# Copojacaab/APDA-FFT

Hardware: NVIDIA B200
Metric: FFT+peak windows/sec at N=4096 (higher is better)
Workload: dtype f32

## Files before the change

apda-fft_b200/csrc/fft_f32_fast.cu:

```cuda
#include <mutex>

#include "fft_f32_fast.cuh"

namespace {

template <int N, int CENTER, bool FULL, bool HALF_OUT>
__global__ void __launch_bounds__(Plan<N>::WPB *(N / 32), Plan<N>::MINB)
fft_f32_fast_kernel(const float *__restrict__ samples, int n_samples, int64_t ld, int64_t batch,
                    const float2 *__restrict__ tw1,
                    const float2 *__restrict__ twu,
                    float2 *__restrict__ spec, const int *__restrict__ nv) {
    using P = Plan<N>;
    constexpr int M = N / 2, R1 = P::R1, R2 = P::R2, R3 = P::R3, T = M / 16, WPB = P::WPB;
    constexpr int S1 = R2 * R3;
    constexpr int LD = S1 + 16 / R1;
    static_assert(R1 * R2 * R3 == M, "plan");
    __shared__ __align__(16) float2 sm[WPB][R1 * LD];
    __shared__ uint32_t sel[WPB][64];
    __shared__ float red[WPB][8];

    const int wslot = threadIdx.x / T;
    const int t = threadIdx.x % T;
    const int64_t win = (int64_t)blockIdx.x * WPB + wslot;
    if (win >= batch) return;
    if (nv && nv[win] != n_samples) return;
    const int64_t winc = win;
    float2 *s = sm[wslot];

    k1_forward<N, CENTER, FULL>(samples, n_samples, ld, winc, tw1, s, sel[wslot], red[wslot], wslot, t);

    float4 *out = reinterpret_cast<float4 *>(spec + win * (int64_t)N);
    const float4 *s4 = reinterpret_cast<const float4 *>(s);
    const float4 *twu4 = reinterpret_cast<const float4 *>(twu);
#pragma unroll
    for (int g = 0; g < (M / 2) / T; ++g) {
        const int p = t + T * g;
        const float4 zk = s4[p];
        const float2 za = s[(M - 2 * p) & (M - 1)];
        const float2 zb = s[M - 2 * p - 1];
        const float4 w = __ldg(twu4 + p);
        const float2 cj = make_float2(1.f, -1.f), ncj = make_float2(-1.f, 1.f), hf = make_float2(0.5f, 0.5f);
        const float2 zk0 = make_float2(zk.x, zk.y), zk1 = make_float2(zk.z, zk.w);
        const float2 s0 = pfma(za, cj, zk0), d0 = pfma(za, ncj, zk0);
        const float2 s1 = pfma(zb, cj, zk1), d1 = pfma(zb, ncj, zk1);
        const float2 t0 = cmul(d0, make_float2(w.x, w.y)), t1 = cmul(d1, make_float2(w.z, w.w));
        const float2 x0 = pfma(s0, hf, t0), x1 = pfma(s1, hf, t1);
        float4 lo4 = make_float4(x0.x, x0.y, x1.x, x1.y);
        if (p == 0) lo4.x = lo4.y = 0.f;
        out[p] = lo4;
        if (!HALF_OUT) {
            const float2 y0 = pfma(s0, hf, make_float2(-t0.x, -t0.y)), y1 = pfma(s1, hf, make_float2(-t1.x, -t1.y));
            out[M / 2 + p] = make_float4(y0.x, y0.y, y1.x, y1.y);
        }
    }
}

struct FastTables {
    float2 *tw1 = nullptr, *twu = nullptr;
};

}

struct FastCache {
    std::map<int64_t, FastTables> tabs;
};
static std::map<apda_ctx *, FastCache> g_fast;
static std::mutex g_fast_mu;
static FastCache &fast_cache_of(apda_ctx *ctx) {
    std::lock_guard<std::mutex> lock(g_fast_mu);
    return g_fast[ctx];
}

template <int N>
static int fast_tables(apda_ctx *ctx, FastTables *out) {
    using P = Plan<N>;
    constexpr int M = N / 2, R1 = P::R1, R2 = P::R2, R3 = P::R3, S1 = R2 * R3;
    auto &cache = fast_cache_of(ctx).tabs;
    auto it = cache.find(N);
    if (it != cache.end()) {
        *out = it->second;
        return APDA_OK;
    }
    const double two_pi = 6.283185307179586476925286766559;
    std::vector<float2> h1((size_t)R1 * S1), hu(M), h2((size_t)R2 * R3);
    for (int k1 = 0; k1 < R1; ++k1)
        for (int c = 0; c < S1; ++c) {
            const double a = -two_pi * (double)((int64_t)k1 * c % M) / (double)M;
            h1[(size_t)k1 * S1 + c] = make_float2((float)cos(a), (float)sin(a));
        }
    for (int k = 0; k < M; ++k) {
        const double a = -two_pi * (double)k / (double)N;
        hu[k] = make_float2((float)(0.5 * sin(a)), (float)(-0.5 * cos(a)));
    }
    for (int k2 = 0; k2 < R2; ++k2)
        for (int n3 = 0; n3 < R3; ++n3) {
            const double a = -two_pi * (double)(k2 * n3) / (double)(R2 * R3);
            h2[(size_t)k2 * R3 + n3] = make_float2((float)cos(a), (float)sin(a));
        }
    FastTables ft;
    APDA_CUDA(cudaMalloc(&ft.tw1, h1.size() * sizeof(float2)));
    APDA_CUDA(cudaMalloc(&ft.twu, hu.size() * sizeof(float2)));
    APDA_CUDA(cudaMemcpy(ft.tw1, h1.data(), h1.size() * sizeof(float2), cudaMemcpyHostToDevice));
    APDA_CUDA(cudaMemcpy(ft.twu, hu.data(), hu.size() * sizeof(float2), cudaMemcpyHostToDevice));
    const void *sym = N == 1024 ? (const void *)c_tw2_1024 : N == 2048 ? (const void *)c_tw2_2048
                    : N == 4096 ? (const void *)c_tw2_4096 : (const void *)c_tw2_8192;
    APDA_CUDA(cudaMemcpyToSymbol(sym, h2.data(), h2.size() * sizeof(float2)));
    cache[N] = ft;
    *out = ft;
    return APDA_OK;
}

template <int N>
static int launch_fast_n(apda_ctx *ctx, cudaStream_t st, const float *d_samples, int64_t n_samples, int64_t ld,
                         int64_t batch, int flags, float *d_spec, const int *d_nv, bool half_out) {
    using P = Plan<N>;
    FastTables ft;
    APDA_TRY(fast_tables<N>(ctx, &ft));
    const int threads = P::WPB * (N / 32);
    const int64_t blocks = (batch + P::WPB - 1) / P::WPB;
    const bool full = n_samples == N && (reinterpret_cast<uintptr_t>(d_samples) & 7u) == 0 && (ld & 1) == 0;
    void (*kern)(const float *, int, int64_t, int64_t, const float2 *, const float2 *, float2 *, const int *);
#define APDA_K1(C, F) (half_out ? fft_f32_fast_kernel<N, C, F, true> : fft_f32_fast_kernel<N, C, F, false>)
    kern = flags == APDA_CENTER_MEDIAN ? (full ? APDA_K1(APDA_CENTER_MEDIAN, true) : APDA_K1(APDA_CENTER_MEDIAN, false))
           : flags == APDA_CENTER_MEAN ? (full ? APDA_K1(APDA_CENTER_MEAN, true) : APDA_K1(APDA_CENTER_MEAN, false))
                                       : (full ? APDA_K1(APDA_CENTER_NONE, true) : APDA_K1(APDA_CENTER_NONE, false));
#undef APDA_K1
    kern<<<(unsigned)blocks, threads, 0, st>>>(d_samples, (int)n_samples, ld, batch, ft.tw1, ft.twu,
                                               reinterpret_cast<float2 *>(d_spec), d_nv);
    ctx->launches++;
    APDA_CUDA(cudaGetLastError());
    return APDA_OK;
}

int fft_f32_fast_get_tables(apda_ctx *ctx, int64_t N, const float2 **tw1, const float2 **twu) {
    FastTables ft;
    switch (N) {
        case 1024: APDA_TRY(fast_tables<1024>(ctx, &ft)); break;
        case 2048: APDA_TRY(fast_tables<2048>(ctx, &ft)); break;
        case 4096: APDA_TRY(fast_tables<4096>(ctx, &ft)); break;
        case 8192: APDA_TRY(fast_tables<8192>(ctx, &ft)); break;
        default: apda_set_error("fft_f32_fast: unsupported N=%lld", (long long)N); return APDA_ERR_UNSUPPORTED;
    }
    *tw1 = ft.tw1;
    *twu = ft.twu;
    return APDA_OK;
}

bool fft_f32_fast_supports(int64_t N) { return N == 1024 || N == 2048 || N == 4096 || N == 8192; }

int launch_fft_f32_fast(apda_ctx *ctx, cudaStream_t st, const float *d_samples, int64_t n_samples, int64_t ld,
                        int64_t batch, int64_t N, int flags, float *d_spec, const int *d_nv, bool half_out) {
    switch (N) {
        case 1024: return launch_fast_n<1024>(ctx, st, d_samples, n_samples, ld, batch, flags, d_spec, d_nv, half_out);
        case 2048: return launch_fast_n<2048>(ctx, st, d_samples, n_samples, ld, batch, flags, d_spec, d_nv, half_out);
        case 4096: return launch_fast_n<4096>(ctx, st, d_samples, n_samples, ld, batch, flags, d_spec, d_nv, half_out);
        case 8192: return launch_fast_n<8192>(ctx, st, d_samples, n_samples, ld, batch, flags, d_spec, d_nv, half_out);
    }
    apda_set_error("fft_f32_fast: unsupported N=%lld", (long long)N);
    return APDA_ERR_UNSUPPORTED;
}

void fft_f32_fast_release(apda_ctx *ctx) {
    std::lock_guard<std::mutex> lock(g_fast_mu);
    auto it = g_fast.find(ctx);
    if (it == g_fast.end()) return;
    for (auto &kv : it->second.tabs) {
        cudaFree(kv.second.tw1);
        cudaFree(kv.second.twu);
    }
    g_fast.erase(it);
}
```

apda-fft_b200/csrc/fft_f32_fast.cuh:

```cuda
#pragma once
#include "common.cuh"

namespace {

__device__ __forceinline__ unsigned long long &u64(float2 &v) { return reinterpret_cast<unsigned long long &>(v); }
__device__ __forceinline__ const unsigned long long &u64(const float2 &v) {
    return reinterpret_cast<const unsigned long long &>(v);
}
__device__ __forceinline__ float2 cadd(float2 a, float2 b) {
    float2 r;
    asm("add.rn.f32x2 %0, %1, %2;" : "=l"(u64(r)) : "l"(u64(a)), "l"(u64(b)));
    return r;
}
__device__ __forceinline__ float2 csub(float2 a, float2 b) {
    float2 r;
    asm("sub.rn.f32x2 %0, %1, %2;" : "=l"(u64(r)) : "l"(u64(a)), "l"(u64(b)));
    return r;
}
__device__ __forceinline__ float2 pmul(float2 a, float2 b) {
    float2 r;
    asm("mul.rn.f32x2 %0, %1, %2;" : "=l"(u64(r)) : "l"(u64(a)), "l"(u64(b)));
    return r;
}
__device__ __forceinline__ float2 pfma(float2 a, float2 b, float2 c) {
    float2 r;
    asm("fma.rn.f32x2 %0, %1, %2, %3;" : "=l"(u64(r)) : "l"(u64(a)), "l"(u64(b)), "l"(u64(c)));
    return r;
}
__device__ __forceinline__ float2 cmul(float2 a, float2 w) {
    return make_float2(fmaf(a.x, w.x, -a.y * w.y), fmaf(a.x, w.y, a.y * w.x));
}

#define SQRT1_2f 0.70710678118654752440f
#define COS_PI_8f 0.92387953251128675613f
#define SIN_PI_8f 0.38268343236508977173f

__device__ __forceinline__ void add_sub_mi(float2 u, float2 d, float2 &plus, float2 &minus) {
    plus = make_float2(u.x + d.y, u.y - d.x);
    minus = make_float2(u.x - d.y, u.y + d.x);
}

__device__ __forceinline__ void fft4(float2 &a0, float2 &a1, float2 &a2, float2 &a3) {
    const float2 t0 = cadd(a0, a2), t1 = csub(a0, a2), t2 = cadd(a1, a3), d = csub(a1, a3);
    a0 = cadd(t0, t2);
    a2 = csub(t0, t2);
    add_sub_mi(t1, d, a1, a3);
}
__device__ __forceinline__ void fft8(float2 *v) {
    float2 e0 = v[0], e1 = v[2], e2 = v[4], e3 = v[6];
    float2 o0 = v[1], o1 = v[3], o2 = v[5], o3 = v[7];
    fft4(e0, e1, e2, e3);
    fft4(o0, o1, o2, o3);
    o1 = pmul(make_float2(o1.x + o1.y, o1.y - o1.x), make_float2(SQRT1_2f, SQRT1_2f));
    o3 = pmul(make_float2(o3.y - o3.x, o3.x + o3.y), make_float2(SQRT1_2f, -SQRT1_2f));
    v[0] = cadd(e0, o0);
    v[4] = csub(e0, o0);
    v[1] = cadd(e1, o1);
    v[5] = csub(e1, o1);
    add_sub_mi(e2, o2, v[2], v[6]);
    v[3] = cadd(e3, o3);
    v[7] = csub(e3, o3);
}
__device__ __forceinline__ void fft16(float2 *v) {
    float2 e[8], o[8];
#pragma unroll
    for (int i = 0; i < 8; ++i) {
        e[i] = v[2 * i];
        o[i] = v[2 * i + 1];
    }
    fft8(e);
    fft8(o);
    const float2 w1 = make_float2(COS_PI_8f, -SIN_PI_8f), w3 = make_float2(SIN_PI_8f, -COS_PI_8f);
    const float2 w5 = make_float2(-SIN_PI_8f, -COS_PI_8f), w7 = make_float2(-COS_PI_8f, -SIN_PI_8f);
    o[1] = cmul(o[1], w1);
    o[2] = pmul(make_float2(o[2].x + o[2].y, o[2].y - o[2].x), make_float2(SQRT1_2f, SQRT1_2f));
    o[3] = cmul(o[3], w3);
    o[5] = cmul(o[5], w5);
    o[6] = pmul(make_float2(o[6].y - o[6].x, o[6].x + o[6].y), make_float2(SQRT1_2f, -SQRT1_2f));
    o[7] = cmul(o[7], w7);
#pragma unroll
    for (int i = 0; i < 8; ++i) {
        if (i == 4) {
            add_sub_mi(e[4], o[4], v[4], v[12]);
        } else {
            v[i] = cadd(e[i], o[i]);
            v[i + 8] = csub(e[i], o[i]);
        }
    }
}
template <int R>
__device__ __forceinline__ void fft_r(float2 *v) {
    if (R == 16) fft16(v);
    else if (R == 8) fft8(v);
    else fft4(v[0], v[1], v[2], v[3]);
}

__constant__ float2 c_tw2_1024[64];
__constant__ float2 c_tw2_2048[64];
__constant__ float2 c_tw2_4096[128];
__constant__ float2 c_tw2_8192[256];
template <int N>
__device__ __forceinline__ const float2 *const_tw2() {
    return N == 1024 ? c_tw2_1024 : N == 2048 ? c_tw2_2048 : N == 4096 ? c_tw2_4096 : c_tw2_8192;
}

#ifndef APDA_K1_MINB_2048
#define APDA_K1_MINB_2048 8
#endif
#ifndef APDA_K1_MINB_1024
#define APDA_K1_MINB_1024 8
#endif
#ifndef APDA_K1_MINB_8192
#define APDA_K1_MINB_8192 4
#endif
#ifndef APDA_K1_MINB
#define APDA_K1_MINB 9
#endif
template <int N>
struct Plan;
template <>
struct Plan<8192> { static constexpr int R1 = 16, R2 = 16, R3 = 16, WPB = 1, MINB = APDA_K1_MINB_8192; };
template <>
struct Plan<4096> { static constexpr int R1 = 16, R2 = 16, R3 = 8, WPB = 1, MINB = APDA_K1_MINB; };
template <>
struct Plan<2048> { static constexpr int R1 = 16, R2 = 8, R3 = 8, WPB = 2, MINB = APDA_K1_MINB_2048; };
template <>
struct Plan<1024> { static constexpr int R1 = 8, R2 = 8, R3 = 8, WPB = 4, MINB = APDA_K1_MINB_1024; };

template <int T>
__device__ __forceinline__ void group_sync(int slot) {
    if (T == 32) __syncwarp();
    else if (slot == 0) asm volatile("bar.sync 1, %0;" ::"n"(T) : "memory");
    else asm volatile("bar.sync 2, %0;" ::"n"(T) : "memory");
}

__device__ __forceinline__ float next_above(float v) {
    float n = key_value(ordered_key(v) + 1u, 0.f);
    if (!(n > v)) n = key_value(ordered_key(v) + 2u, 0.f);
    return n;
}

__device__ __noinline__ float2 bracket_minmax(float2 a0, float2 a1, float2 a2, float2 a3, float2 a4, float2 a5, float2 a6,
                                              float2 a7, float2 a8, float2 a9, float2 a10, float2 a11, float2 a12, float2 a13,
                                              float2 a14, float2 a15, unsigned inb) {
    const float2 a[16] = {a0, a1, a2, a3, a4, a5, a6, a7, a8, a9, a10, a11, a12, a13, a14, a15};
    float vmin = CUDART_INF_F, vmax = -CUDART_INF_F;
#pragma unroll
    for (int i = 0; i < 16; ++i) {
        if (inb & (0x80000000u >> (2 * i))) {
            vmin = fminf(vmin, a[i].x);
            vmax = fmaxf(vmax, a[i].x);
        }
        if (inb & (0x80000000u >> (2 * i + 1))) {
            vmin = fminf(vmin, a[i].y);
            vmax = fmaxf(vmax, a[i].y);
        }
    }
#pragma unroll
    for (int o = 16; o > 0; o >>= 1) {
        vmin = fminf(vmin, __shfl_xor_sync(0xffffffffu, vmin, o));
        vmax = fmaxf(vmax, __shfl_xor_sync(0xffffffffu, vmax, o));
    }
    return make_float2(vmin, vmax);
}

constexpr int kTightenFrom = 4;
template <int T, bool FULL, typename Reload>
__device__ float select_median(const float2 (&v2)[16], int n_valid, uint32_t *sh , int t, int slot,
                               Reload reload ) {
#define VAL(i) (((i) & 1) ? v2[(i) >> 1].y : v2[(i) >> 1].x)
    constexpr int NW = (T + 31) / 32;
    const int lane = t & 31, warp = t >> 5;
    const int r_lo = (n_valid - 1) >> 1, r_hi = n_valid >> 1;
    float *shf = reinterpret_cast<float *>(sh);

    {
        float s1 = 0.f, s2 = 0.f;
        int cntv = 0;
#pragma unroll
        for (int c = 0; c < 16; c += 4) {
#pragma unroll
            for (int h = 0; h < 2; ++h) {
                const float raw = h ? v2[c].y : v2[c].x;
                const bool ok = FULL || raw < CUDART_INF_F;
                const float x = ok ? raw : 0.f;
                s1 += x;
                s2 = fmaf(x, x, s2);
                cntv += ok;
            }
        }
#pragma unroll
        for (int o = 16; o > 0; o >>= 1) {
            s1 += __shfl_xor_sync(0xffffffffu, s1, o);
            s2 += __shfl_xor_sync(0xffffffffu, s2, o);
        }
        if (!FULL) cntv = __reduce_add_sync(0xffffffffu, cntv);
        if (lane == 0) {
            shf[warp] = s1;
            shf[8 + warp] = s2;
            if (!FULL) sh[16 + warp] = (uint32_t)cntv;
        }
        if (t == 0) sh[48] = 0;
    }
    group_sync<T>(slot);
    float mean, sd;
    {
        float s1 = 0.f, s2 = 0.f;
        int cntv = FULL ? 8 * T : 0;
#pragma unroll
        for (int w = 0; w < NW; ++w) {
            s1 += shf[w];
            s2 += shf[8 + w];
            if (!FULL) cntv += (int)sh[16 + w];
        }
        const float inv = rcp_approx((float)max(cntv, 1));
        mean = s1 * inv;
        sd = sqrt_approx(fmaxf(fmaf(-mean, mean, s2 * inv), 0.f));
    }
    const float inv_density = fmaxf(2.5f * sd, 1e-30f) * rcp_approx((float)n_valid);

    float lo = -CUDART_INF_F, hi = CUDART_INF_F;
    int c_lo = 0, c_hi = n_valid;
    unsigned mask_lo = 0u, mask_hi = 0xffffffffu;
    if (!FULL) {
        mask_hi = 0u;
#pragma unroll
        for (int i = 0; i < 32; ++i) mask_hi = (mask_hi << 1) | (VAL(i) < CUDART_INF_F ? 1u : 0u);
    }
    float pivot = mean;
    for (int round = 0;; ++round) {
        if (round > 0) {
            if (c_hi - c_lo <= 32) break;
            if (round >= kTightenFrom) {
                const float2 mm = bracket_minmax(v2[0], v2[1], v2[2], v2[3], v2[4], v2[5], v2[6], v2[7], v2[8], v2[9], v2[10],
                                                 v2[11], v2[12], v2[13], v2[14], v2[15], ~mask_lo & mask_hi);
                if (lane == 0) {
                    shf[warp] = mm.x;
                    shf[8 + warp] = mm.y;
                }
                group_sync<T>(slot);
                float vmin = shf[0], vmax = shf[8];
#pragma unroll
                for (int w = 1; w < NW; ++w) {
                    vmin = fminf(vmin, shf[w]);
                    vmax = fmaxf(vmax, shf[8 + w]);
                }
                if (vmin == vmax) {
                    group_sync<T>(slot);
                    return vmin;
                }
                lo = vmin;
                hi = next_above(vmax);
            }
            const float lo_next = lo > -CUDART_INF_F ? next_above(lo) : -3.4028234e38f;
            if (!(lo_next < hi)) break;
            const float want = (float)r_lo + 0.5f;
            if (lo == -CUDART_INF_F) {
                pivot = hi - 1.5f * fmaxf((float)c_hi - want, 1.f) * inv_density * (float)(1 << min(round - 1, 20));
            } else if (hi == CUDART_INF_F) {
                pivot = lo + 1.5f * fmaxf(want - (float)c_lo, 1.f) * inv_density * (float)(1 << min(round - 1, 20));
            } else if (round % 3 == 2) {
                const uint32_t a = ordered_key(lo), b = ordered_key(hi);
                pivot = key_value(a + ((b - a) >> 1), 0.f);
            } else {
                pivot = lo + (hi - lo) * __fdividef(want - (float)c_lo, (float)(c_hi - c_lo));
            }
            if (!(pivot > lo)) pivot = lo_next;
            if (!(pivot < hi)) pivot = lo_next;
        }
        unsigned signs = 0;
        const float2 pv = make_float2(pivot, pivot);
#pragma unroll
        for (int i = 0; i < 16; ++i) {
            const float2 d = csub(v2[i], pv);
            signs = __funnelshift_l(__float_as_uint(d.x), signs, 1);
            signs = __funnelshift_l(__float_as_uint(d.y), signs, 1);
        }
        int cnt = __popc(signs);
        cnt = __reduce_add_sync(0xffffffffu, cnt);
        uint32_t *cslot = sh + 32 + 8 * (round & 1);
        if (lane == 0) cslot[warp] = (uint32_t)cnt;
        group_sync<T>(slot);
        int tot = 0;
#pragma unroll
        for (int w = 0; w < NW; ++w) tot += (int)cslot[w];
        if (tot <= r_lo) {
            lo = pivot;
            c_lo = tot;
            mask_lo = signs;
        } else if (tot > r_hi) {
            hi = pivot;
            c_hi = tot;
            mask_hi = signs;
        } else {
            float below = -CUDART_INF_F, above = CUDART_INF_F;
#pragma unroll
            for (int i = 0; i < 32; ++i) {
                if (VAL(i) < pivot) below = fmaxf(below, VAL(i));
                else above = fminf(above, VAL(i));
            }
#pragma unroll
            for (int o = 16; o > 0; o >>= 1) {
                below = fmaxf(below, __shfl_xor_sync(0xffffffffu, below, o));
                above = fminf(above, __shfl_xor_sync(0xffffffffu, above, o));
            }
            if (lane == 0) {
                shf[warp] = below;
                shf[8 + warp] = above;
            }
            group_sync<T>(slot);
#pragma unroll
            for (int w = 0; w < NW; ++w) {
                below = fmaxf(below, shf[w]);
                above = fminf(above, shf[8 + w]);
            }
            group_sync<T>(slot);
            return (below + above) * 0.5f;
        }
    }
    if (c_hi - c_lo > 32) {
        group_sync<T>(slot);
        return lo;
    }
    for (unsigned inb = ~mask_lo & mask_hi; inb; ) {
        const int q = __clz(inb);
        inb &= ~(0x80000000u >> q);
        const uint32_t pos = atomicAdd(&sh[48], 1u);
        if (pos < 32u) shf[pos] = reload(q);
    }
    group_sync<T>(slot);
    const int cnt = (int)sh[48];
    if (warp == 0) {
        float med;
        if (cnt > 32) {
            med = lo;
        } else {
            const float mine = lane < cnt ? shf[lane] : CUDART_INF_F;
            int rank = 0;
            for (int j = 0; j < cnt; ++j) {
                const float other = shf[j];
                rank += (other < mine) || (other == mine && j < lane);
            }
            const uint32_t m_lo = __ballot_sync(0xffffffffu, lane < cnt && rank == r_lo - c_lo);
            const uint32_t m_hi = __ballot_sync(0xffffffffu, lane < cnt && rank == r_hi - c_lo);
            const float a = __shfl_sync(0xffffffffu, mine, __ffs(m_lo) - 1);
            const float b = __shfl_sync(0xffffffffu, mine, __ffs(m_hi) - 1);
            med = (a + b) * 0.5f;
        }
        if (lane == 0) shf[49] = med;
    }
    group_sync<T>(slot);
    return shf[49];
}
#undef VAL

template <int N, int CENTER, bool FULL, int PF_AHEAD = 0>
__device__ __forceinline__ void k1_forward(const float *__restrict__ samples, const int n_samples, const int64_t ld,
                                           const int64_t winc, const float2 *__restrict__ tw1, float2 *s, uint32_t *sel_w,
                                           float *red_w, const int wslot, const int t, const int64_t pf_batch = 0) {
    constexpr int center = CENTER;
    using P = Plan<N>;
    constexpr int M = N / 2, R1 = P::R1, R2 = P::R2, R3 = P::R3, T = M / 16;
    constexpr int S1 = R2 * R3;
    constexpr int LD = S1 + 16 / R1;
    constexpr int G1 = 16 / R1, G2 = 16 / R2, G3 = 16 / R3;
    float2 v[16];
    const float *x = samples + winc * ld;
    const float2 *z = reinterpret_cast<const float2 *>(x);
    const bool full = FULL;
#pragma unroll
    for (int g = 0; g < G1; ++g) {
        const int c = t + T * g;
#pragma unroll
        for (int n1 = 0; n1 < R1; ++n1) {
            const int zi = n1 * S1 + c;
            float2 val;
            if (FULL) {
                val = __ldg(z + zi);
            } else {
                val.x = (2 * zi < n_samples) ? __ldg(x + 2 * zi) : 0.f;
                val.y = (2 * zi + 1 < n_samples) ? __ldg(x + 2 * zi + 1) : 0.f;
            }
            v[g * R1 + n1] = val;
        }
    }
    if (APDA_L2_PREFETCH && PF_AHEAD > 0) {
        const int64_t wn = winc + (int64_t)sm_count_reg() * PF_AHEAD;
        if (wn < pf_batch) l2_prefetch_span(samples + wn * ld, n_samples * (int)sizeof(float), t, T);
    }
    float shift = 0.f;
    if (center == APDA_CENTER_MEDIAN) {
        if (!full) {
#pragma unroll
            for (int g = 0; g < G1; ++g)
#pragma unroll
                for (int n1 = 0; n1 < R1; ++n1) {
                    const int zi = n1 * S1 + t + T * g;
                    if (2 * zi >= n_samples) v[g * R1 + n1].x = CUDART_INF_F;
                    if (2 * zi + 1 >= n_samples) v[g * R1 + n1].y = CUDART_INF_F;
                }
        }
        auto reload = [&](int q) {
            const int j = q >> 1;
            return __ldg(x + 2 * ((j % R1) * S1 + t + T * (j / R1)) + (q & 1));
        };
        shift = select_median<T, FULL>(v, n_samples, sel_w, t, wslot, reload);
        if (!full) {
#pragma unroll
            for (int i = 0; i < 16; ++i) {
                if (v[i].x == CUDART_INF_F) v[i].x = 0.f;
                if (v[i].y == CUDART_INF_F) v[i].y = 0.f;
            }
        }
    } else if (center == APDA_CENTER_MEAN) {
        float acc = 0.f;
#pragma unroll
        for (int i = 0; i < 16; ++i) acc += v[i].x + v[i].y;
#pragma unroll
        for (int o = 16; o > 0; o >>= 1) acc += __shfl_xor_sync(0xffffffffu, acc, o);
        if ((t & 31) == 0) red_w[t >> 5] = acc;
        group_sync<T>(wslot);
        float tot = 0.f;
#pragma unroll
        for (int w = 0; w < (T + 31) / 32; ++w) tot += red_w[w];
        shift = tot / (float)n_samples;
    }
#pragma unroll
    for (int g = 0; g < G1; ++g) {
        const int c = t + T * g;
        if (center != APDA_CENTER_NONE) {
#pragma unroll
            for (int n1 = 0; n1 < R1; ++n1) {
                const int zi = n1 * S1 + c;
                if (full) {
                    v[g * R1 + n1] = csub(v[g * R1 + n1], make_float2(shift, shift));
                } else {
                    if (2 * zi < n_samples) v[g * R1 + n1].x -= shift;
                    if (2 * zi + 1 < n_samples) v[g * R1 + n1].y -= shift;
                }
            }
        }
        fft_r<R1>(v + g * R1);
        s[c] = v[g * R1];
#pragma unroll
        for (int k1 = 1; k1 < R1; ++k1) s[k1 * LD + c] = cmul(v[g * R1 + k1], __ldg(tw1 + k1 * S1 + c));
    }
    group_sync<T>(wslot);

    const float2 *tw2 = const_tw2<N>();
#pragma unroll
    for (int g = 0; g < G2; ++g) {
        const int w = t + T * g;
        const int k1 = w % R1, n3 = w / R1;
        float2 *col = s + k1 * LD + n3;
#pragma unroll
        for (int n2 = 0; n2 < R2; ++n2) v[g * R2 + n2] = col[n2 * R3];
        fft_r<R2>(v + g * R2);
        col[0] = v[g * R2];
#pragma unroll
        for (int k2 = 1; k2 < R2; ++k2) col[k2 * R3] = cmul(v[g * R2 + k2], tw2[k2 * R3 + n3]);
    }
    group_sync<T>(wslot);

#pragma unroll
    for (int g = 0; g < G3; ++g) {
        const int w = t + T * g;
        const int k1 = w % R1, k2 = w / R1;
        const float2 *row = s + k1 * LD + k2 * R3;
#pragma unroll
        for (int n3 = 0; n3 < R3; ++n3) v[g * R3 + n3] = row[n3];
        fft_r<R3>(v + g * R3);
    }
    group_sync<T>(wslot);
#pragma unroll
    for (int g = 0; g < G3; ++g) {
        const int w = t + T * g;
#pragma unroll
        for (int k3 = 0; k3 < R3; ++k3) s[w + R1 * R2 * k3] = v[g * R3 + k3];
    }
    group_sync<T>(wslot);

}

}
```

apda-fft_b200/csrc/fused_f32.cu:

```cuda
#include <mutex>

#include "fft_f32_fast.cuh"
#include "peaks_fast.cuh"

int fft_f32_fast_get_tables(apda_ctx *ctx, int64_t N, const float2 **tw1, const float2 **twu);

namespace {

template <int N>
struct FusedLayout {
    using P = Plan<N>;
    static constexpr int M = N / 2, T = M / 16;
    static constexpr int FFT_BYTES = (int)sizeof(float2) * P::R1 * (P::R2 * P::R3 + 16 / P::R1);
    static constexpr int MAG_BYTES = K3M<M>::MAGW * (int)sizeof(float);
    static constexpr int BYTES = FFT_BYTES + MAG_BYTES + 128;
    static constexpr int SLOT_CAP = M / 5 + 8;
    static_assert(2 * T * (int)sizeof(float) + SLOT_CAP * (int)sizeof(Slot) <= FFT_BYTES, "tail scratch must fit the FFT buffer");
};

#ifndef APDA_FUSED_MINB
#define APDA_FUSED_MINB 8
#endif
template <int N, int CENTER, bool FULL, bool FLEX>
__global__ void __launch_bounds__(N / 32, (N == 4096 ? APDA_FUSED_MINB : N < 4096 ? 1024 / (N / 32) / 2 : 2))
fused_f32_kernel(const float *__restrict__ samples, int n_samples, int64_t ld, int64_t batch,
                 const float2 *__restrict__ tw1, const float2 *__restrict__ twu, double df_all,
                 const double *__restrict__ d_fs, int k, unsigned char *__restrict__ recs) {
    using L = FusedLayout<N>;
    using Q = K3M<N / 2>;
    constexpr int M = N / 2, T = M / 16;
    extern __shared__ __align__(16) unsigned char dyn_smem[];
    float2 *s = reinterpret_cast<float2 *>(dyn_smem);
    float *mags = reinterpret_cast<float *>(dyn_smem + L::FFT_BYTES);
    unsigned char *rec_s = dyn_smem + L::FFT_BYTES + L::MAG_BYTES;
    __shared__ uint32_t sel[64];
    __shared__ float red[8];
    __shared__ double stat[2 * (T / 32 > 0 ? T / 32 : 1)];
    __shared__ int ctl[2];
    const int t = threadIdx.x, lane = t & 31, warp = t >> 5;
    const int64_t win = blockIdx.x;
    if (win >= batch) return;
    if (t == 0) ctl[0] = ctl[1] = 0;

    k1_forward<N, CENTER, FULL, (N == 4096 ? APDA_FUSED_MINB : N < 4096 ? 1024 / (N / 32) / 2 : 2)>(
        samples, n_samples, ld, win, tw1, s, sel, red, 0, t, batch);

    if (t < 16) reinterpret_cast<uint64_t *>(rec_s)[t] = (t % 3 == 1) ? 0x00000000ffffffffull : 0ull;
    const float4 *s4 = reinterpret_cast<const float4 *>(s);
    const float4 *twu4 = reinterpret_cast<const float4 *>(twu);
    float sum = 0.f, sumsq = 0.f;
#pragma unroll
    for (int g = 0; g < (M / 2) / T; ++g) {
        const int p = t + T * g;
        const float4 zk = s4[p];
        const float2 za = s[(M - 2 * p) & (M - 1)];
        const float2 zb = s[M - 2 * p - 1];
        const float4 w = __ldg(twu4 + p);
        const float2 cj = make_float2(1.f, -1.f), ncj = make_float2(-1.f, 1.f), hf = make_float2(0.5f, 0.5f);
        const float2 zk0 = make_float2(zk.x, zk.y), zk1 = make_float2(zk.z, zk.w);
        const float2 s0 = pfma(za, cj, zk0), d0 = pfma(za, ncj, zk0);
        const float2 s1 = pfma(zb, cj, zk1), d1 = pfma(zb, ncj, zk1);
        const float2 t0 = cmul(d0, make_float2(w.x, w.y)), t1 = cmul(d1, make_float2(w.z, w.w));
        float2 x0 = pfma(s0, hf, t0);
        const float2 x1 = pfma(s1, hf, t1);
        if (p == 0) x0 = make_float2(0.f, 0.f);
        const float p0 = fmaf(x0.x, x0.x, x0.y * x0.y), p1 = fmaf(x1.x, x1.x, x1.y * x1.y);
        const float m0 = sqrt_fast(p0), m1 = sqrt_fast(p1);
        sum += m0 + m1;
        sumsq += p0 + p1;
        *reinterpret_cast<float2 *>(mags + Q::addr(2 * p)) = make_float2(m0, m1);
    }
    double S = (double)sum, Qs = (double)sumsq;
#pragma unroll
    for (int o = 16; o > 0; o >>= 1) {
        S += __shfl_xor_sync(0xffffffffu, S, o);
        Qs += __shfl_xor_sync(0xffffffffu, Qs, o);
    }
    constexpr int NW = T / 32 > 0 ? T / 32 : 1;
    if (lane == 0) {
        stat[warp] = S;
        stat[NW + warp] = Qs;
    }
    group_sync<T>(0);
    S = 0.0;
    Qs = 0.0;
#pragma unroll
    for (int w = 0; w < NW; ++w) {
        S += stat[w];
        Qs += stat[NW + w];
    }
    const double nn = (double)M;
    const double mean = S / nn;
    const double var = (Qs - S * S / nn) / (nn - 1.0);
    const double sd = var > 0.0 ? sqrt(var) : 0.0;
    const double thr = mean + 2.0 * sd;
    const float thr_f = __double2float_rd(thr);
    const double df = d_fs ? div_rn(d_fs[win], (double)N) : df_all;
    float *cmaxs = reinterpret_cast<float *>(s), *cmins = cmaxs + T;
    Slot *slots = reinterpret_cast<Slot *>(cmins + T);
    k3_tail_mw<M, FLEX, T>(mags, cmaxs, cmins, slots, L::SLOT_CAP, ctl, rec_s, sd, thr_f, df, k, t, win, recs);
}

template <int N>
int upload_tw2(int device) {
    static std::vector<int> done;
    static std::mutex mu;
    std::lock_guard<std::mutex> lock(mu);
    for (int d : done)
        if (d == device) return APDA_OK;
    using P = Plan<N>;
    constexpr int R2 = P::R2, R3 = P::R3;
    const double two_pi = 6.283185307179586476925286766559;
    std::vector<float2> h2((size_t)R2 * R3);
    for (int k2 = 0; k2 < R2; ++k2)
        for (int n3 = 0; n3 < R3; ++n3) {
            const double a = -two_pi * (double)(k2 * n3) / (double)(R2 * R3);
            h2[(size_t)k2 * R3 + n3] = make_float2((float)cos(a), (float)sin(a));
        }
    const void *sym = N == 1024 ? (const void *)c_tw2_1024 : N == 2048 ? (const void *)c_tw2_2048
                    : N == 4096 ? (const void *)c_tw2_4096 : (const void *)c_tw2_8192;
    APDA_CUDA(cudaMemcpyToSymbol(sym, h2.data(), h2.size() * sizeof(float2)));
    done.push_back(device);
    return APDA_OK;
}

template <int N>
int launch_fused_n(apda_ctx *ctx, cudaStream_t st, const float *d_samples, int64_t n_samples, int64_t ld, int64_t batch,
                   int flags, int flexible, double fs, const double *d_fs, int k, void *d_rec) {
    const float2 *tw1, *twu;
    APDA_TRY(fft_f32_fast_get_tables(ctx, N, &tw1, &twu));
    APDA_TRY(upload_tw2<N>(ctx->device));
    const bool full = n_samples == N && (reinterpret_cast<uintptr_t>(d_samples) & 7u) == 0 && (ld & 1) == 0;
    const bool med = flags == APDA_CENTER_MEDIAN;
    void (*kern)(const float *, int, int64_t, int64_t, const float2 *, const float2 *, double, const double *, int,
                 unsigned char *);
#define PICK(C, F, X) fused_f32_kernel<N, C, F, X>
    if (flexible) {
        kern = med ? (full ? PICK(APDA_CENTER_MEDIAN, true, true) : PICK(APDA_CENTER_MEDIAN, false, true))
                   : (full ? PICK(APDA_CENTER_MEAN, true, true) : PICK(APDA_CENTER_MEAN, false, true));
    } else {
        kern = med ? (full ? PICK(APDA_CENTER_MEDIAN, true, false) : PICK(APDA_CENTER_MEDIAN, false, false))
                   : (full ? PICK(APDA_CENTER_MEAN, true, false) : PICK(APDA_CENTER_MEAN, false, false));
    }
#undef PICK
    const size_t smem = FusedLayout<N>::BYTES;
    APDA_FUNC_SMEM(ctx, kern, smem);
    kern<<<(unsigned)batch, N / 32, smem, st>>>(d_samples, (int)n_samples, ld, batch, tw1, twu, fs / (double)N, d_fs, k,
                                            reinterpret_cast<unsigned char *>(d_rec));
    ctx->launches++;
    APDA_CUDA(cudaGetLastError());
    return APDA_OK;
}

}

int launch_fused_f32(apda_ctx *ctx, cudaStream_t st, const float *d_samples, int64_t n_samples, int64_t ld, int64_t batch,
                     int64_t N, int flags, int flexible, double fs, const double *d_fs, int k, void *d_rec) {
    switch (N) {
        case 1024: return launch_fused_n<1024>(ctx, st, d_samples, n_samples, ld, batch, flags, flexible, fs, d_fs, k, d_rec);
        case 2048: return launch_fused_n<2048>(ctx, st, d_samples, n_samples, ld, batch, flags, flexible, fs, d_fs, k, d_rec);
        case 4096: return launch_fused_n<4096>(ctx, st, d_samples, n_samples, ld, batch, flags, flexible, fs, d_fs, k, d_rec);
        case 8192: return launch_fused_n<8192>(ctx, st, d_samples, n_samples, ld, batch, flags, flexible, fs, d_fs, k, d_rec);
    }
    apda_set_error("fused_f32: unsupported N=%lld", (long long)N);
    return APDA_ERR_UNSUPPORTED;
}
```

Baseline: 80.33 million.

## Pair pass-3 rows per thread to fuse real-FFT unpack without shared round-trip

When the plan's last radix is 8, each thread now takes the mirror row (RR - t) as its second pass-3 row. That lets it run the real-to-complex unpack directly from registers, skipping the shared-memory store, two group syncs and the reload in the standalone FFT kernel. The radix-16 twiddle multiplies are also rewritten as a packed FMA with precomputed rotated constants. The trade-off is scattered float2 stores instead of float4 stores, and the fused FFT+peak kernel only changes its call signature.

Result: faster. 81.64 million (median of 6 runs) (+1.6%).

```diff
diff --git a/apda-fft_b200/csrc/fft_f32_fast.cu b/apda-fft_b200/csrc/fft_f32_fast.cu
--- a/apda-fft_b200/csrc/fft_f32_fast.cu
+++ b/apda-fft_b200/csrc/fft_f32_fast.cu
@@ -27,7 +27,39 @@
     const int64_t winc = win;
     float2 *s = sm[wslot];
 
-    k1_forward<N, CENTER, FULL>(samples, n_samples, ld, winc, tw1, s, sel[wslot], red[wslot], wslot, t);
+    constexpr bool PAIRED = R3 == 8;
+    float2 v[16];
+    k1_forward<N, CENTER, FULL, 0, PAIRED>(v, samples, n_samples, ld, winc, tw1, s, sel[wslot], red[wslot], wslot, t);
+
+    const float2 cj = make_float2(1.f, -1.f), ncj = make_float2(-1.f, 1.f), hf = make_float2(0.5f, 0.5f);
+    if constexpr (PAIRED) {
+        constexpr int RR = R1 * R2;
+        float2 *out = spec + win * (int64_t)N;
+        const auto bin = [&](float2 zk, float2 zp, int k, bool zero) {
+            const float2 wt = __ldg(twu + k);
+            const float2 s0 = pfma(zp, cj, zk), d0 = pfma(zp, ncj, zk);
+            const float2 t0 = cmul(d0, wt);
+            float2 x0 = pfma(s0, hf, t0);
+            if (zero) x0 = make_float2(0.f, 0.f);
+            out[k] = x0;
+            if (!HALF_OUT) out[M + k] = pfma(s0, hf, make_float2(-t0.x, -t0.y));
+        };
+        if (t != 0) {
+            const int w2 = RR - t;
+#pragma unroll
+            for (int k3 = 0; k3 < R3; ++k3) {
+                bin(v[k3], v[2 * R3 - 1 - k3], t + RR * k3, false);
+                bin(v[2 * R3 - 1 - k3], v[k3], w2 + RR * (R3 - 1 - k3), false);
+            }
+        } else {
+#pragma unroll
+            for (int k3 = 0; k3 < R3; ++k3) {
+                bin(v[k3], v[(R3 - k3) & (R3 - 1)], RR * k3, k3 == 0);
+                bin(v[R3 + k3], v[2 * R3 - 1 - k3], RR / 2 + RR * k3, false);
+            }
+        }
+        return;
+    }
 
     float4 *out = reinterpret_cast<float4 *>(spec + win * (int64_t)N);
     const float4 *s4 = reinterpret_cast<const float4 *>(s);
@@ -39,7 +71,6 @@
         const float2 za = s[(M - 2 * p) & (M - 1)];
         const float2 zb = s[M - 2 * p - 1];
         const float4 w = __ldg(twu4 + p);
-        const float2 cj = make_float2(1.f, -1.f), ncj = make_float2(-1.f, 1.f), hf = make_float2(0.5f, 0.5f);
         const float2 zk0 = make_float2(zk.x, zk.y), zk1 = make_float2(zk.z, zk.w);
         const float2 s0 = pfma(za, cj, zk0), d0 = pfma(za, ncj, zk0);
         const float2 s1 = pfma(zb, cj, zk1), d1 = pfma(zb, ncj, zk1);
diff --git a/apda-fft_b200/csrc/fft_f32_fast.cuh b/apda-fft_b200/csrc/fft_f32_fast.cuh
--- a/apda-fft_b200/csrc/fft_f32_fast.cuh
+++ b/apda-fft_b200/csrc/fft_f32_fast.cuh
@@ -29,6 +29,9 @@
 }
 __device__ __forceinline__ float2 cmul(float2 a, float2 w) {
     return make_float2(fmaf(a.x, w.x, -a.y * w.y), fmaf(a.x, w.y, a.y * w.x));
+}
+__device__ __forceinline__ float2 cmul2(float2 a, float2 w, float2 wr) {
+    return pfma(make_float2(a.x, a.x), w, pmul(make_float2(a.y, a.y), wr));
 }
 
 #define SQRT1_2f 0.70710678118654752440f
@@ -72,12 +75,14 @@
     fft8(o);
     const float2 w1 = make_float2(COS_PI_8f, -SIN_PI_8f), w3 = make_float2(SIN_PI_8f, -COS_PI_8f);
     const float2 w5 = make_float2(-SIN_PI_8f, -COS_PI_8f), w7 = make_float2(-COS_PI_8f, -SIN_PI_8f);
-    o[1] = cmul(o[1], w1);
+    const float2 r1 = make_float2(SIN_PI_8f, COS_PI_8f), r3 = make_float2(COS_PI_8f, SIN_PI_8f);
+    const float2 r5 = make_float2(COS_PI_8f, -SIN_PI_8f), r7 = make_float2(SIN_PI_8f, -COS_PI_8f);
+    o[1] = cmul2(o[1], w1, r1);
     o[2] = pmul(make_float2(o[2].x + o[2].y, o[2].y - o[2].x), make_float2(SQRT1_2f, SQRT1_2f));
-    o[3] = cmul(o[3], w3);
-    o[5] = cmul(o[5], w5);
+    o[3] = cmul2(o[3], w3, r3);
+    o[5] = cmul2(o[5], w5, r5);
     o[6] = pmul(make_float2(o[6].y - o[6].x, o[6].x + o[6].y), make_float2(SQRT1_2f, -SQRT1_2f));
-    o[7] = cmul(o[7], w7);
+    o[7] = cmul2(o[7], w7, r7);
 #pragma unroll
     for (int i = 0; i < 8; ++i) {
         if (i == 4) {
@@ -354,17 +359,24 @@
 }
 #undef VAL
 
-template <int N, int CENTER, bool FULL, int PF_AHEAD = 0>
-__device__ __forceinline__ void k1_forward(const float *__restrict__ samples, const int n_samples, const int64_t ld,
-                                           const int64_t winc, const float2 *__restrict__ tw1, float2 *s, uint32_t *sel_w,
-                                           float *red_w, const int wslot, const int t, const int64_t pf_batch = 0) {
+template <int N>
+__device__ __forceinline__ int pair_row(int t) {
+    constexpr int RR = Plan<N>::R1 * Plan<N>::R2;
+    return t ? RR - t : RR / 2;
+}
+
+template <int N, int CENTER, bool FULL, int PF_AHEAD = 0, bool PAIRED = false>
+__device__ __forceinline__ void k1_forward(float2 (&v)[16], const float *__restrict__ samples, const int n_samples,
+                                           const int64_t ld, const int64_t winc, const float2 *__restrict__ tw1, float2 *s,
+                                           uint32_t *sel_w, float *red_w, const int wslot, const int t,
+                                           const int64_t pf_batch = 0) {
     constexpr int center = CENTER;
     using P = Plan<N>;
     constexpr int M = N / 2, R1 = P::R1, R2 = P::R2, R3 = P::R3, T = M / 16;
     constexpr int S1 = R2 * R3;
     constexpr int LD = S1 + 16 / R1;
     constexpr int G1 = 16 / R1, G2 = 16 / R2, G3 = 16 / R3;
-    float2 v[16];
+    static_assert(!PAIRED || (G3 == 2 && R1 * R2 == 2 * T), "row pairing needs two pass-3 rows per thread");
     const float *x = samples + winc * ld;
     const float2 *z = reinterpret_cast<const float2 *>(x);
     const bool full = FULL;
@@ -464,13 +476,14 @@
 
 #pragma unroll
     for (int g = 0; g < G3; ++g) {
-        const int w = t + T * g;
+        const int w = PAIRED && g == 1 ? pair_row<N>(t) : t + T * g;
         const int k1 = w % R1, k2 = w / R1;
         const float2 *row = s + k1 * LD + k2 * R3;
 #pragma unroll
         for (int n3 = 0; n3 < R3; ++n3) v[g * R3 + n3] = row[n3];
         fft_r<R3>(v + g * R3);
     }
+    if (PAIRED) return;
     group_sync<T>(wslot);
 #pragma unroll
     for (int g = 0; g < G3; ++g) {
@@ -479,7 +492,6 @@
         for (int k3 = 0; k3 < R3; ++k3) s[w + R1 * R2 * k3] = v[g * R3 + k3];
     }
     group_sync<T>(wslot);
-
-}
-
-}
+}
+
+}
diff --git a/apda-fft_b200/csrc/fused_f32.cu b/apda-fft_b200/csrc/fused_f32.cu
--- a/apda-fft_b200/csrc/fused_f32.cu
+++ b/apda-fft_b200/csrc/fused_f32.cu
@@ -42,8 +42,9 @@
     if (win >= batch) return;
     if (t == 0) ctl[0] = ctl[1] = 0;
 
+    float2 v[16];
     k1_forward<N, CENTER, FULL, (N == 4096 ? APDA_FUSED_MINB : N < 4096 ? 1024 / (N / 32) / 2 : 2)>(
-        samples, n_samples, ld, win, tw1, s, sel, red, 0, t, batch);
+        v, samples, n_samples, ld, win, tw1, s, sel, red, 0, t, batch);
 
     if (t < 16) reinterpret_cast<uint64_t *>(rec_s)[t] = (t % 3 == 1) ? 0x00000000ffffffffull : 0ull;
     const float4 *s4 = reinterpret_cast<const float4 *>(s);
```
